# SCUT-BIP-Lab/SplatCo

Measured on AMD Instinct MI355X. Metric: rasterizer fwd+bwd Msplats/s @1080p; PSNR-match vs ref, higher is better.
Workload: dtype f32; 1 GPU; cfg1: 1M synthetic Gaussians (seed 0), 1 view 1920x1080 per GPU, GaussianRasterizer forward+backward, colors_precomp + scale/rotation path; gaussians=1000000, image=1920x1080, visible=1000000, parallelism=1 view per GPU (mv sharding)

## Files before the change

splatco_amd/csrc/binning.hip:

```cpp
#include "common.h"

namespace scr {

template <int THREADS>
__device__ __forceinline__ uint32_t block_exclusive_scan(uint32_t v, uint32_t* lds_waves ,
                                                         uint32_t& block_total) {
    const int lane = threadIdx.x & (WAVE - 1), w = threadIdx.x / WAVE;
    uint32_t inc = v;
#pragma unroll
    for (int d = 1; d < WAVE; d <<= 1) {
        uint32_t n = __shfl_up(inc, d, WAVE);
        if (lane >= d) inc += n;
    }
    if (lane == WAVE - 1) lds_waves[w] = inc;
    __syncthreads();
    uint32_t base = 0, tot = 0;
#pragma unroll
    for (int k = 0; k < THREADS / WAVE; ++k) {
        uint32_t s = lds_waves[k];
        if (k < w) base += s;
        tot += s;
    }
    block_total = tot;
    __syncthreads();
// ... 17 lines not shown
            uint32_t ex = block_exclusive_scan<1024>(v, lds, tot);
            if (i < nblk) block_sums[i] = (uint32_t)carry + ex;
            carry += tot;
            mine += v;
        }
#pragma unroll
        for (int d = WAVE / 2; d > 0; d >>= 1) mine += (unsigned long long)__shfl_down((long long)mine, d, WAVE);
        __syncthreads();
        if ((threadIdx.x & (WAVE - 1)) == 0) wide[threadIdx.x / WAVE] = mine;
        __syncthreads();
        if (threadIdx.x == 0) {
            carry = 0;
            for (int w = 0; w < 1024 / WAVE; ++w) carry += wide[w];
            total[0] = carry;
            if (mailbox) {
                mailbox[0] = carry;
                __threadfence_system();
                mailbox[1] = seq;
            }
        }
    } else {
        uint32_t carry = 0, mx = 0;
        for (uint32_t base = 0; base < tiles; base += 1024) {
            uint32_t i = base + threadIdx.x;
            uint32_t v = i < tiles ? tile_count[i] : 0u, tot;
            uint32_t ex = block_exclusive_scan<1024>(v, lds, tot);
            if (i < tiles) {
                ranges[2 * i] = carry + ex;
                ranges[2 * i + 1] = carry + ex + v;
                cursor[i] = 0;
            }
            carry += tot;
            mx = max(mx, v);
        }
#pragma unroll
        for (int d = 32; d > 0; d >>= 1) mx = max(mx, (uint32_t)__shfl_xor((int)mx, d, WAVE));
        __syncthreads();
        if ((threadIdx.x & 63) == 0) lds[threadIdx.x >> 6] = mx;
        __syncthreads();
        if (threadIdx.x == 0) {
            uint32_t m = 0;
            for (int w = 0; w < 1024 / WAVE; ++w) m = max(m, lds[w]);
            total[1] = m;
            total[2] = 0;
            if (mailbox) {
                mailbox[2] = (unsigned long long)m | (total[3] << 32);
                __threadfence_system();
                mailbox[3] = seq;
            }
        }
    }
}

template <bool LDS_HIST>
__global__ void __launch_bounds__(BIN_THREADS)
scatter_kernel(int64_t P, int gx, int tiles, const float4* __restrict__ rec, uint2* __restrict__ gm_base,
               uint32_t* __restrict__ live_bits, const uint32_t* __restrict__ tiles_touched, const uint32_t* __restrict__ block_prefix,
               uint32_t* __restrict__ point_offsets, const uint32_t* __restrict__ ranges,
               uint32_t* __restrict__ cursor, unsigned long long* __restrict__ keys,
               const unsigned long long* __restrict__ total, unsigned long long cap_instances) {
    extern __shared__ __attribute__((aligned(16))) uint32_t hist[];
    __shared__ uint32_t lds[BIN_THREADS / WAVE + 1];
    if (total[0] > cap_instances) return;
    if (LDS_HIST) {
        for (int t = threadIdx.x; t < tiles; t += BIN_THREADS) hist[t] = 0;
        __syncthreads();
    }
    uint32_t off[BIN_ROUNDS], tts[BIN_ROUNDS], rlo[BIN_ROUNDS], rhi[BIN_ROUNDS], dbits[BIN_ROUNDS];
    uint32_t carry = block_prefix[blockIdx.x];
#pragma unroll
    for (int r = 0; r < BIN_ROUNDS; ++r) {
        const int64_t i = (int64_t)blockIdx.x * BIN_GPW + r * BIN_THREADS + threadIdx.x;
        const uint32_t tt = i < P ? tiles_touched[i] : 0u;
        uint32_t tot;
        off[r] = carry + block_exclusive_scan<BIN_THREADS>(tt, lds, tot);
        carry += tot;
        tts[r] = tt;
        rlo[r] = rhi[r] = dbits[r] = 0;
        if (i < P) point_offsets[i] = off[r] + tt;
        if (tt) {
            const float4 r2 = rec[3 * i + 2];
            dbits[r] = __float_as_uint(r2.y);
            rlo[r] = __float_as_uint(r2.z);
            rhi[r] = __float_as_uint(r2.w);
            const uint32_t x0 = rlo[r] & 0xffff, y0 = rlo[r] >> 16, rw = (rhi[r] & 0xffff) - x0;
            gm_base[i] = make_uint2(off[r] - y0 * rw - x0, rw);
            if (LDS_HIST)
                for (int ty = rlo[r] >> 16; ty < (int)(rhi[r] >> 16); ++ty)
                    for (int tx = rlo[r] & 0xffff; tx < (int)(rhi[r] & 0xffff); ++tx) atomicAdd(&hist[ty * gx + tx], 1u);
        }
    }
    if (LDS_HIST) {
        __syncthreads();
        for (int t = threadIdx.x; t < tiles; t += BIN_THREADS) {
            const uint32_t c = hist[t];
            if (c) hist[t] = ranges[2 * t] + atomicAdd(&cursor[t], c);
        }
        __syncthreads();
    }
#pragma unroll
    for (int r = 0; r < BIN_ROUNDS; ++r) {
        if (!tts[r]) continue;
        const int64_t i = (int64_t)blockIdx.x * BIN_GPW + r * BIN_THREADS + threadIdx.x;
        const uint32_t klo = (uint32_t)i << 4;
        const float4 r0 = rec[3 * i], r1 = rec[3 * i + 1];
        const unsigned long long khi = (unsigned long long)dbits[r] << 32;
        uint32_t live = 0, kbit = 1;
        for (int ty = rlo[r] >> 16; ty < (int)(rhi[r] >> 16); ++ty)
            for (int tx = rlo[r] & 0xffff; tx < (int)(rhi[r] & 0xffff); ++tx) {
                const uint32_t t = (uint32_t)(ty * gx + tx);
                const uint32_t slot = LDS_HIST ? atomicAdd(&hist[t], 1u) : ranges[2 * t] + atomicAdd(&cursor[t], 1u);
                const uint32_t qm = quadrant_mask(r0, r1, tx * TILE, ty * TILE);
                keys[slot] = khi | klo | qm;
                live |= qm ? kbit : 0u;
                kbit <<= 1;
            }
        live_bits[i] = live;
    }
}

template <int D>
__device__ __forceinline__ uint32_t lane_xor(uint32_t v) {
    if constexpr (D == 1) {
        return (uint32_t)__builtin_amdgcn_mov_dpp((int)v, 0xB1, 0xf, 0xf, true);
    } else if constexpr (D == 2) {
        return (uint32_t)__builtin_amdgcn_mov_dpp((int)v, 0x4E, 0xf, 0xf, true);
    } else if constexpr (D == 4) {
        int t = __builtin_amdgcn_update_dpp((int)v, (int)v, 0x104, 0xf, 0x5, false);
        return (uint32_t)__builtin_amdgcn_update_dpp(t, (int)v, 0x114, 0xf, 0xA, false);
    } else if constexpr (D == 8) {
        int t = __builtin_amdgcn_update_dpp((int)v, (int)v, 0x108, 0xf, 0x3, false);
        return (uint32_t)__builtin_amdgcn_update_dpp(t, (int)v, 0x118, 0xf, 0xC, false);
    } else if constexpr (D == 16) {
        auto r = __builtin_amdgcn_permlane16_swap(v, v, false, false);
        return sel(0xFFFF0000FFFF0000ull, r[0], r[1]);
    } else {
        auto r = __builtin_amdgcn_permlane32_swap(v, v, false, false);
        return sel(0xFFFFFFFF00000000ull, r[0], r[1]);
    }
}

constexpr unsigned long long lanes_with_bit_clear(int bit) {
    unsigned long long m = 0;
    for (int l = 0; l < 64; ++l)
        if ((l & bit) == 0) m |= 1ull << l;
// ... 357 lines not shown
    {
        auto keyA = [&](uint32_t i) { return buf[wg_slot((int)i)]; };
        auto keyB = [&](uint32_t j) { return buf[wg_slot((int)(na + j))]; };
        uint32_t a = d0 > nb ? d0 - nb : 0u, b = min(d0, na);
        while (a < b) {
            const uint32_t mid = (a + b) >> 1;
            if (keyA(mid) < keyB(d0 - mid - 1)) a = mid + 1;
            else b = mid;
        }
        uint32_t ia = a, ib = d0 - a;
        unsigned long long x = ia < na ? keyA(ia) : ~0ull, y = ib < nb ? keyB(ib) : ~0ull;
#pragma unroll
        for (int k = 0; k < PER; ++k) {
            const bool takeA = x < y;
            outk[k] = takeA ? x : y;
            if (takeA) {
                ++ia;
                x = ia < na ? keyA(ia) : ~0ull;
            } else {
                ++ib;
                y = ib < nb ? keyB(ib) : ~0ull;
            }
        }
    }
    __syncthreads();
#pragma unroll
    for (int k = 0; k < PER; ++k)
        if (d0 + k < tot) buf[wg_slot((int)(d0 + k))] = outk[k];
    __syncthreads();
    if (pass + 1 == merge_passes_needed(n)) {
        const FinalLists fl{gm_base, point_list, gm_index, qmask, t % gx, t / gx};
        for (uint32_t e = threadIdx.x; e < tot; e += 4 * 256)
            fl.template write_batch<4>(lo + pairbase + s0, e, 256u, tot, [&](uint32_t i, int) { return (uint32_t)buf[wg_slot((int)i)]; });
    } else {
        unsigned long long* out = dst + lo + pairbase + s0;
        for (uint32_t e = threadIdx.x; e < tot; e += 256) out[e] = buf[wg_slot((int)e)];
    }
}

void launch_plan_scans(int64_t P, const KSettings& ks, const GeomView& gv, unsigned long long* mailbox,
                       unsigned long long seq, hipStream_t st) {
    Grid g(ks.H, ks.W);
    uint32_t nb = (uint32_t)((P + BIN_GPW - 1) / BIN_GPW);
    plan_scan_kernel<<<2, 1024, 0, st>>>(nb, gv.block_sums, gv.total, (uint32_t)g.tiles, gv.tile_count,
                                         gv.ranges, gv.cursor, mailbox, seq);
}

void launch_scatter(int64_t P, const KSettings& ks, const GeomView& gv, const BinView& bv, unsigned long long cap_instances,
                    hipStream_t st) {
    if (P <= 0) return;
    Grid g(ks.H, ks.W);
    const unsigned nb = (unsigned)((P + BIN_GPW - 1) / BIN_GPW);
    allow_dynamic_lds((const void*)scatter_kernel<true>, LDS_HIST_MAX_TILES * 4);
    if (g.tiles <= LDS_HIST_MAX_TILES)
        scatter_kernel<true><<<nb, BIN_THREADS, (size_t)g.tiles * 4, st>>>(
            P, g.gx, g.tiles, gv.rec, gv.gm_base, gv.live_bits, gv.tiles_touched, gv.block_sums, gv.point_offsets, gv.ranges,
            gv.cursor, bv.keys, gv.total, cap_instances);
    else
        scatter_kernel<false><<<nb, BIN_THREADS, 0, st>>>(
            P, g.gx, g.tiles, gv.rec, gv.gm_base, gv.live_bits, gv.tiles_touched, gv.block_sums, gv.point_offsets, gv.ranges,
            gv.cursor, bv.keys, gv.total, cap_instances);
}

void launch_tile_sort(const KSettings& ks, const GeomView& gv, const BinView& bv, int64_t max_tile_instances,
                      bool with_gm_index, hipStream_t st) {
    uint32_t* const gm_index = with_gm_index ? bv.gm_index : nullptr;
    Grid g(ks.H, ks.W);
    const unsigned gt = (unsigned)xcd_grid(g.tiles);
    if (max_tile_instances <= 0) return;
    tile_sort_wave_kernel<<<gt, 64, 0, st>>>(g.tiles, g.gx, gv.ranges, bv.keys, gv.gm_base, bv.point_list, gm_index,
                                             bv.qmask);
    if (max_tile_instances <= WAVE_SORT_MAX) return;
    const unsigned chunks = (unsigned)((max_tile_instances + WG_SORT_MAX - 1) / WG_SORT_MAX);
    const size_t lds = (size_t)(WG_SORT_MAX + WG_SORT_MAX / 16) * 8;
    allow_dynamic_lds((const void*)tile_sort_wg_kernel, lds);
    tile_sort_wg_kernel<<<dim3(gt, chunks), WG_SORT_THREADS, lds, st>>>(g.tiles, g.gx, gv.ranges, bv.keys, gv.gm_base, bv.point_list,
                                                                        gm_index, bv.qmask);
    if (chunks <= 1) return;
    unsigned passes = 0;
    while ((1u << passes) < chunks) ++passes;
    const unsigned segs = (unsigned)((max_tile_instances + MP_SEG - 1) / MP_SEG);
    for (unsigned p = 0; p < passes; ++p) {
        const unsigned long long* src = (p & 1u) ? bv.keys2 : bv.keys;
        unsigned long long* dst = (p & 1u) ? bv.keys : bv.keys2;
        tile_merge_path_kernel<<<dim3(gt, segs), 256, 0, st>>>(g.tiles, g.gx, p, gv.ranges, src, dst, gv.gm_base,
                                                               bv.point_list, gm_index, bv.qmask);
    }
}

}
```

splatco_amd/csrc/capi.hip:

```cpp
#include <stdarg.h>
#include <stdio.h>
#include <string.h>

#include "common.h"
#include "adam.h"
#include "tv.h"
#include <chrono>
#include <map>
#include <mutex>
#include <utility>
#include <cstring>

using namespace scr;

static thread_local char g_err[512] = "";
namespace scr {
int g_force_deep_lists = -1;

void allow_dynamic_lds(const void* kernel, size_t bytes) {
    if (bytes <= 65536) return;
    static std::mutex mu;
    static std::map<std::pair<int, const void*>, size_t> granted;
    int dev = 0;
    (void)hipGetDevice(&dev);
    std::lock_guard<std::mutex> lk(mu);
    size_t& have = granted[{dev, kernel}];
    if (bytes <= have) return;
    if (hipFuncSetAttribute(kernel, hipFuncAttributeMaxDynamicSharedMemorySize, (int)bytes) == hipSuccess) have = bytes;
    (void)hipGetLastError();
}
}

static int fail(const char* fmt, ...) {
    va_list ap;
    va_start(ap, fmt);
    vsnprintf(g_err, sizeof(g_err), fmt, ap);
    va_end(ap);
    return 1;
}

#define HIP_TRY(expr)                                                                      \
    do {                                                                                   \
        hipError_t e_ = (expr);                                                            \
        if (e_ != hipSuccess) return fail("%s failed: %s", #expr, hipGetErrorString(e_)); \
    } while (0)

#define CHECK_LAUNCH(name, debug, st)                                                      \
    do {                                                                                   \
        hipError_t e_ = hipGetLastError();                                                 \
        if (e_ != hipSuccess) return fail("launch of %s failed: %s", name, hipGetErrorString(e_)); \
        if (debug) {                                                                       \
            e_ = hipStreamSynchronize(st);                                                 \
            if (e_ != hipSuccess) return fail("%s faulted: %s", name, hipGetErrorString(e_)); \
        }                                                                                  \
    } while (0)

#include <dlfcn.h>
#include <atomic>
#include <vector>
namespace {
struct ProfRec { int idx; hipEvent_t a, b; };
unsigned g_prof_mask = 0;
unsigned g_prof_stride = 1;
unsigned g_prof_seen[32] = {};
std::vector<ProfRec> g_prof_recs;
std::vector<hipEvent_t> g_prof_pool;
hipEvent_t prof_event() {
    hipEvent_t e;
    if (!g_prof_pool.empty()) { e = g_prof_pool.back(); g_prof_pool.pop_back(); return e; }
    (void)hipEventCreate(&e);
// ... 372 lines not shown
    if (check_settings(settings)) return 1;
    if (P < 0) return fail("P < 0");
    const bool camera = dL_dviewmatrix || dL_dprojmatrix || dL_dcampos;
    if (P == 0) {
        if (dL_dviewmatrix) HIP_TRY(hipMemsetAsync(dL_dviewmatrix, 0, 16 * sizeof(float), (hipStream_t)stream));
        if (dL_dprojmatrix) HIP_TRY(hipMemsetAsync(dL_dprojmatrix, 0, 16 * sizeof(float), (hipStream_t)stream));
        if (dL_dcampos) HIP_TRY(hipMemsetAsync(dL_dcampos, 0, 3 * sizeof(float), (hipStream_t)stream));
        return 0;
    }
    if (plan_flags & ~(int64_t)(SCR_PLAN_NONFINITE_COLOUR | SCR_PLAN_LARGE_RECTS)) return fail("plan_flags %lld: not a value scr_forward_plan returned", (long long)plan_flags);
    if (!geom_buf || !binning_buf || !image_buf || !dL_dcolor || !scratch) return fail("NULL buffer");
    if (!means3D || !radii || !dL_dmeans3D || !dL_dmeans2D || !dL_dopacity) return fail("NULL argument");
    if (shs ? !dL_dsh : !dL_dcolors) return fail("colour gradient output missing");
    if (cov3D_precomp ? !dL_dcov3D : !(dL_dscales && dL_drotations && scales && rotations))
        return fail("covariance gradient output missing");
    hipStream_t st = (hipStream_t)stream;
    KSettings ks = ksettings(settings);
    GeomView gv = geom_view(geom_buf, P, ks.H, ks.W);
    BinView bv = bin_view((void*)binning_buf, I, 0);
    ImgView iv = img_view(image_buf, ks.H, ks.W);
    static std::atomic<unsigned long long> stamp_counter{0x5ca1ab1e00000000ull};
    const unsigned long long stamp = ++stamp_counter;
    float* const grad_z = (I > 0 && (dL_ddepth || dL_dalpha)) ? (float*)((char*)scratch + grad_rec_bytes(I)) : nullptr;
    float* const cam_partials = camera ? (float*)((char*)scratch + grad_rec_bytes(I) + grad_z_bytes(I)) : nullptr;
    if (settings->debug) {
        unsigned long long dev_flags = 0;
        HIP_TRY(hipMemcpyAsync(&dev_flags, gv.total + 3, 8, hipMemcpyDeviceToHost, st));
        HIP_TRY(hipStreamSynchronize(st));
        if ((long long)dev_flags != (long long)plan_flags)
            return fail("plan_flags %lld passed to scr_backward, but the forward pass of this geom_buf raised %llu", (long long)plan_flags, dev_flags);
    }
    if (I > 0) {
        launch_zero_far_records(P, gv, (GradRec*)scratch, grad_z, st);
        CHECK_LAUNCH("zero_far_records_kernel", settings->debug, st);
        { ProfScope ps_(SCR_PROF_BLEND_BACKWARD, st);
          launch_blend_backward(ks, gv, bv, iv, dL_dcolor, dL_ddepth, dL_dalpha, (GradRec*)scratch, grad_z, stamp, deep_lists(I, Grid(ks.H, ks.W).tiles),
                                record_flags(I, Grid(ks.H, ks.W).tiles), (plan_flags & SCR_PLAN_NONFINITE_COLOUR) != 0, st); }
        CHECK_LAUNCH("blend_backward_kernel", settings->debug, st);
    }
    { ProfScope ps_(SCR_PROF_PREPROCESS_BACKWARD, st);
      launch_preprocess_backward(P, M, means3D, scales, rotations, cov3D_precomp, shs, ks, radii, gv, bv,
                                 (const GradRec*)scratch, grad_z, iv.cut_key, stamp, record_flags(I, Grid(ks.H, ks.W).tiles), dL_dmeans3D, dL_dmeans2D, shs ? nullptr : dL_dcolors,
                                 shs ? dL_dsh : nullptr, dL_dopacity, cov3D_precomp ? nullptr : dL_dscales,
                                 cov3D_precomp ? nullptr : dL_drotations, cov3D_precomp ? dL_dcov3D : nullptr, cam_partials, st); }
    CHECK_LAUNCH("preprocess_backward_kernel", settings->debug, st);
    if (camera) {
        launch_camera_grad_finish(P, cam_partials, dL_dviewmatrix, dL_dprojmatrix, dL_dcampos, st);
        CHECK_LAUNCH("camera_grad_finish_kernel", settings->debug, st);
    }
    return 0;
}

int scr_debug_force_deep_lists(int mode) {
    if (mode < -1 || mode > 1) return fail("scr_debug_force_deep_lists: -1 (automatic), 0 or 1");
    scr::g_force_deep_lists = mode;
    return 0;
}

int scr_debug_get(int which, int64_t P, int64_t I, int32_t H, int32_t W, const void* geom_buf,
                  const void* binning_buf, const void* image_buf, void* out, void* stream) {
    SCR_MARK_FN;
    hipStream_t st = (hipStream_t)stream;
    Grid g(H, W);
    const void* src = nullptr;
    size_t bytes = 0;
    if (which <= SCR_DBG_RANGES || which == SCR_DBG_SPLAT_RECORDS) {
        if (!geom_buf) return fail("geom_buf is NULL");
        GeomView gv = geom_view((void*)geom_buf, P, H, W);
        if (which == SCR_DBG_TILES_TOUCHED) { src = gv.tiles_touched; bytes = (size_t)P * 4; }
        else if (which == SCR_DBG_POINT_OFFSETS) { src = gv.point_offsets; bytes = (size_t)P * 4; }
        else if (which == SCR_DBG_RANGES) { src = gv.ranges; bytes = (size_t)g.tiles * 8; }
        else { src = gv.rec; bytes = (size_t)P * REC_F * 4; }
    } else if (which == SCR_DBG_POINT_LIST) {
        if (!binning_buf) return fail("binning_buf is NULL");
        src = bin_view((void*)binning_buf, I, 0).point_list;
        bytes = (size_t)I * 4;
    } else if (which == SCR_DBG_QMASK || which == SCR_DBG_GM_INDEX) {
        if (!binning_buf) return fail("binning_buf is NULL");
        BinView bv = bin_view((void*)binning_buf, I, 0);
        if (which == SCR_DBG_GM_INDEX && deep_lists(I, g.tiles))
            return fail("gm_index is not materialised for deep tile lists (I > 8192 per tile on average)");
        src = which == SCR_DBG_QMASK ? (const void*)bv.qmask : (const void*)bv.gm_index;
        bytes = which == SCR_DBG_QMASK ? (size_t)I : (size_t)I * 4;
    } else if (which == SCR_DBG_N_CONTRIB || which == SCR_DBG_FINAL_T) {
        if (!image_buf) return fail("image_buf is NULL");
        ImgView iv = img_view((void*)image_buf, H, W);
        src = which == SCR_DBG_N_CONTRIB ? (const void*)iv.n_contrib : (const void*)iv.final_T;
        bytes = (size_t)H * W * 4;
    } else {
        return fail("unknown debug selector %d", which);
    }
    if (bytes) HIP_TRY(hipMemcpyAsync(out, src, bytes, hipMemcpyDeviceToDevice, st));
    return 0;
}

static inline size_t expand_nwg(int64_t n) { return (size_t)((n + 1023) / 1024); }

size_t scr_expand_scratch_bytes(int64_t n) { return align_up((expand_nwg(n) + 1) * 4) + 256; }

int scr_expand_plan(int64_t n, const float* neural_opacity, void* scratch, int64_t* num_selected_host,
                    void* stream) {
    SCR_MARK_FN;
    if (!num_selected_host) return fail("num_selected_host is NULL");
    *num_selected_host = 0;
    if (n < 0) return fail("n < 0");
    if (n == 0) return 0;
    if (!neural_opacity || !scratch) return fail("NULL argument");
    if (n >= (1ll << 31)) return fail("more than 2^31 candidates");
// ... 793 lines not shown
```

splatco_amd/csrc/common.h:

```cpp
#pragma once
#include <hip/hip_runtime.h>
#include <stdint.h>

#include "../../include/splatco_raster.h"

namespace scr {

__host__ __device__ __forceinline__ uint32_t sat_add_u32(uint32_t a, uint32_t b) {
    const uint32_t s = a + b;
    return s < a ? 0xFFFFFFFFu : s;
}


constexpr int TILE = SCR_TILE;
constexpr int TILE_PIX = TILE * TILE;
constexpr int WAVE = 64;
constexpr int NUM_XCD = 8;
constexpr int PRE_BLOCK = 256;
constexpr int BIN_THREADS = 1024;
constexpr int BIN_ROUNDS = 4;
constexpr int BIN_GPW = BIN_THREADS * BIN_ROUNDS;
constexpr int LDS_HIST_MAX_TILES = 40000;
constexpr int ID_BITS = 28;
constexpr int WG_SORT_MAX = 8192;
constexpr int REC_F = 12;
constexpr int GRAD_F = 9;

inline __host__ __device__ size_t align_up(size_t x, size_t a = 256) { return (x + a - 1) / a * a; }

struct Grid {
    int W, H, gx, gy, tiles;
    __host__ __device__ Grid(int H_, int W_)
        : W(W_), H(H_), gx((W_ + TILE - 1) / TILE), gy((H_ + TILE - 1) / TILE), tiles(gx * gy) {}
};

struct GeomView {
    float4* rec;
    uint32_t* tiles_touched;
    uint32_t* point_offsets;
    uint8_t* clamped;
    uint2* gm_base;
    uint32_t* live_bits;
    uint8_t* has_rec;
    uint32_t* block_sums;
    uint32_t* tile_count;
    uint32_t* ranges;
    uint32_t* cursor;
    int64_t P;
    unsigned long long* total;
    size_t bytes;
};

inline __host__ GeomView geom_view(void* base, int64_t P, int H, int W) {
    Grid g(H, W);
    char* p = (char*)base;
    size_t off = 0;
    GeomView v;
    auto take = [&](size_t n) { char* q = p ? p + off : nullptr; off += align_up(n); return q; };
    size_t nblk = (size_t)((P + BIN_GPW - 1) / BIN_GPW);
    v.rec = (float4*)take((size_t)P * REC_F * 4);
    v.tiles_touched = (uint32_t*)take((size_t)P * 4);
    v.point_offsets = (uint32_t*)take((size_t)P * 4);
    v.clamped = (uint8_t*)take((size_t)P);
    v.gm_base = (uint2*)take((size_t)P * 8);
    v.live_bits = (uint32_t*)take((size_t)P * 4);
    v.has_rec = (uint8_t*)take((size_t)P);
    v.block_sums = (uint32_t*)take((nblk + 1) * 4);
    v.tile_count = (uint32_t*)take((size_t)g.tiles * 4);
    v.ranges = (uint32_t*)take((size_t)g.tiles * 8);
    v.cursor = (uint32_t*)take((size_t)g.tiles * 4);
    v.total = (unsigned long long*)take(128);
    v.bytes = off;
    v.P = P;
    return v;
}

extern int g_force_deep_lists;
inline __host__ bool deep_lists(int64_t I, int tiles) {
    return g_force_deep_lists >= 0 ? g_force_deep_lists != 0 : I > (int64_t)8192 * tiles;
}

constexpr int FLAGS_MIN_MEAN = 2048;
inline __host__ bool record_flags(int64_t I, int tiles) {
    return g_force_deep_lists >= 0 ? g_force_deep_lists != 0 : I > (int64_t)FLAGS_MIN_MEAN * tiles;
}

struct BinView {
    unsigned long long* keys;
    uint32_t* point_list;
    uint32_t* gm_index;
    uint8_t* qmask;
    unsigned long long* keys2;
    size_t bytes;
};

inline __host__ BinView bin_view(void* base, int64_t I, int64_t max_tile_instances) {
    char* p = (char*)base;
    size_t off = 0;
    BinView v;
    auto take = [&](size_t n) { char* q = p ? p + off : nullptr; off += align_up(n); return q; };
    size_t n = (size_t)(I > 0 ? I : 1);
    v.keys = (unsigned long long*)take(n * 8);
    v.point_list = (uint32_t*)take(n * 4);
    v.gm_index = (uint32_t*)take(n * 4);
    v.qmask = (uint8_t*)take(n);
    const bool merge = max_tile_instances > WG_SORT_MAX;
    v.keys2 = merge ? (unsigned long long*)take(n * 8) : nullptr;
    v.bytes = off;
    return v;
}

struct __attribute__((packed, aligned(4))) GradQuad { float x, y, z, w; };
struct __attribute__((packed, aligned(4))) GradRec { GradQuad a, b; float c; };
static_assert(sizeof(GradRec) == 36, "36-byte gradient records");
inline __host__ size_t grad_rec_bytes(int64_t I) { return align_up((size_t)(I > 0 ? I : 1) * sizeof(GradRec)); }
inline __host__ size_t grad_z_bytes(int64_t I) { return align_up((size_t)(I > 0 ? I : 1) * sizeof(float)); }

struct ImgView {
    float* final_T;
    uint32_t* n_contrib;
    unsigned long long* cut_key;
    size_t bytes;
};

// ... 311 lines not shown
```

splatco_amd/csrc/preprocess.hip:

```cpp
#include "common.h"

namespace scr {

struct Proj {
    float t[3];
    float hx, hy, hw;
    float cov[6];
    float txc, tyc;
    bool clx, cly;
    float T[2][3];
    float a, b, c;
};

__device__ __forceinline__ void xform3(const float* __restrict__ M, float x, float y, float z, int i,
                                       float& out) {
    out = ((M[i] * x + M[4 + i] * y) + M[8 + i] * z) + M[12 + i];
}

__device__ __forceinline__ void rotmat(const float q[4], float R[3][3]) {
    float r = q[0], x = q[1], y = q[2], z = q[3];
    R[0][0] = 1.0f - 2.0f * (y * y + z * z);
    R[0][1] = 2.0f * (x * y - r * z);
    R[0][2] = 2.0f * (x * z + r * y);
    R[1][0] = 2.0f * (x * y + r * z);
// ... 122 lines not shown
}

__global__ void __launch_bounds__(256) mark_visible_kernel(int64_t P, const float* __restrict__ means3D,
                                                           const float* __restrict__ V,
                                                           uint8_t* __restrict__ out) {
    int64_t i = (int64_t)blockIdx.x * 256 + threadIdx.x;
    if (i >= P) return;
    float tz;
    xform3(V, means3D[3 * i], means3D[3 * i + 1], means3D[3 * i + 2], 2, tz);
    out[i] = tz > 0.2f;
}

__device__ static const float SH_C0 = 0.28209479177387814f;
__device__ static const float SH_C1 = 0.4886025119029199f;
__device__ static const float SH_C2[5] = {1.0925484305920792f, -1.0925484305920792f, 0.31539156525252005f,
                                          -1.0925484305920792f, 0.5462742152960396f};
__device__ static const float SH_C3[7] = {-0.5900435899266435f, 2.890611442640554f, -0.4570457994644658f,
                                          0.3731763325901154f,  -0.4570457994644658f, 1.445305721320277f,
                                          -0.5900435899266435f};

__device__ __forceinline__ void sh_to_rgb(int deg, const float* __restrict__ sh, float x, float y,
                                          float z, float rgb[3], uint8_t& clampbits) {
    clampbits = 0;
#pragma unroll
    for (int c = 0; c < 3; ++c) {
#define SHV(k) sh[(k)*3 + c]
        float res = SH_C0 * SHV(0);
        if (deg > 0) {
            res = res - SH_C1 * y * SHV(1) + SH_C1 * z * SHV(2) - SH_C1 * x * SHV(3);
            if (deg > 1) {
                float xx = x * x, yy = y * y, zz = z * z, xy = x * y, yz = y * z, xz = x * z;
                res = res + SH_C2[0] * xy * SHV(4) + SH_C2[1] * yz * SHV(5) +
                      SH_C2[2] * (2.0f * zz - xx - yy) * SHV(6) + SH_C2[3] * xz * SHV(7) +
                      SH_C2[4] * (xx - yy) * SHV(8);
                if (deg > 2) {
                    res = res + SH_C3[0] * y * (3.0f * xx - yy) * SHV(9) + SH_C3[1] * xy * z * SHV(10) +
                          SH_C3[2] * y * (4.0f * zz - xx - yy) * SHV(11) +
                          SH_C3[3] * z * (2.0f * zz - 3.0f * xx - 3.0f * yy) * SHV(12) +
                          SH_C3[4] * x * (4.0f * zz - xx - yy) * SHV(13) + SH_C3[5] * z * (xx - yy) * SHV(14) +
                          SH_C3[6] * x * (xx - 3.0f * yy) * SHV(15);
                }
            }
        }
#undef SHV
        res += 0.5f;
        if (res < 0.0f) {
            clampbits |= (uint8_t)(1u << c);
            res = 0.0f;
        }
        rgb[c] = res;
    }
}

template <bool LDS_HIST>
__global__ void __launch_bounds__(BIN_THREADS)
preprocess_kernel(int64_t P, int M, const float* __restrict__ means3D, const float* __restrict__ scales,
                  const float* __restrict__ rotations, const float* __restrict__ cov3D,
                  const float* __restrict__ opacities, const float* __restrict__ shs,
                  const float* __restrict__ colors, KSettings ks, int tiles, float4* __restrict__ rec,
                  uint32_t* __restrict__ tiles_touched, uint8_t* __restrict__ clamped,
                  uint32_t* __restrict__ block_sums, uint32_t* __restrict__ tile_count,
                  int32_t* __restrict__ radii, unsigned long long* __restrict__ plan_flags) {
    extern __shared__ __attribute__((aligned(16))) uint32_t hist[];
    __shared__ uint32_t wave_sum[BIN_THREADS / WAVE];
    if (LDS_HIST) {
        for (int t = threadIdx.x; t < tiles; t += BIN_THREADS) hist[t] = 0;
        __syncthreads();
    }
    const int gx = (ks.W + TILE - 1) / TILE;
    uint32_t tsum = 0;
    for (int r = 0; r < BIN_ROUNDS; ++r) {
        const int64_t i = (int64_t)blockIdx.x * BIN_GPW + r * BIN_THREADS + threadIdx.x;
        if (i >= P) break;
        uint32_t tt = 0;
        Proj ps;
        Foot ft;
        bool vis = project(i, means3D, scales, rotations, cov3D, ks, ps, ft);
        if (vis) {
            float a = ps.a, b = ps.b, c = ps.c;
            float Qxx = c * ft.det_inv, Qxy = -b * ft.det_inv, Qyy = a * ft.det_inv;
            float rgb[3];
            uint8_t cb = 0;
            if (colors) {
                rgb[0] = colors[3 * i];
                rgb[1] = colors[3 * i + 1];
                rgb[2] = colors[3 * i + 2];
            } else {
                float dx = means3D[3 * i] - ks.campos[0], dy = means3D[3 * i + 1] - ks.campos[1],
                      dz = means3D[3 * i + 2] - ks.campos[2];
                float n = sqrtf((dx * dx + dy * dy) + dz * dz);
                sh_to_rgb(ks.sh_degree, shs + (size_t)i * M * 3, dx / n, dy / n, dz / n, rgb, cb);
            }
            if (clamped) clamped[i] = cb;
            tt = (uint32_t)((ft.rmaxx - ft.rminx) * (ft.rmaxy - ft.rminy));
            const unsigned long long w_nf = lanes(nonfinite3(rgb[0], rgb[1], rgb[2])), w_big = lanes(tt > 32u);
            if ((w_nf | w_big) != 0ull) {
                const unsigned long long active = lanes(true);
                if ((int)__builtin_amdgcn_mbcnt_hi(~0u, __builtin_amdgcn_mbcnt_lo(~0u, 0u)) == __builtin_ctzll(active))
                    atomicOr(plan_flags, (unsigned long long)((w_nf ? SCR_PLAN_NONFINITE_COLOUR : 0) | (w_big ? SCR_PLAN_LARGE_RECTS : 0)));
            }
            uint32_t rlo = (uint32_t)ft.rminx | ((uint32_t)ft.rminy << 16);
            uint32_t rhi = (uint32_t)ft.rmaxx | ((uint32_t)ft.rmaxy << 16);
            rec[3 * i + 0] = make_float4(ft.mx, ft.my, -0.5f * Qxx, -Qxy);
            rec[3 * i + 1] = make_float4(-0.5f * Qyy, opacities[i], rgb[0], rgb[1]);
            rec[3 * i + 2] = make_float4(rgb[2], ps.t[2], __uint_as_float(rlo), __uint_as_float(rhi));
            radii[i] = ft.radius;
            for (int ty = ft.rminy; ty < ft.rmaxy; ++ty)
                for (int tx = ft.rminx; tx < ft.rmaxx; ++tx) {
                    if (LDS_HIST) atomicAdd(&hist[ty * gx + tx], 1u);
                    else atomicAdd(&tile_count[ty * gx + tx], 1u);
                }
        } else {
            radii[i] = 0;
            if (clamped) clamped[i] = 0;
        }
        tiles_touched[i] = tt;
        tsum = sat_add_u32(tsum, tt);
    }
    uint32_t s = tsum;
#pragma unroll
    for (int d = WAVE / 2; d > 0; d >>= 1) s = sat_add_u32(s, (uint32_t)__shfl_down(s, d, WAVE));
    if ((threadIdx.x & (WAVE - 1)) == 0) wave_sum[threadIdx.x / WAVE] = s;
    __syncthreads();
    if (threadIdx.x == 0) {
        uint32_t tot = 0;
#pragma unroll
        for (int w = 0; w < BIN_THREADS / WAVE; ++w) tot = sat_add_u32(tot, wave_sum[w]);
        block_sums[blockIdx.x] = tot;
    }
    if (LDS_HIST)
        for (int t = threadIdx.x; t < tiles; t += BIN_THREADS) {
            const uint32_t c = hist[t];
            if (c) atomicAdd(&tile_count[t], c);
        }
}

constexpr int CAM_VALUES = 27, CAM_ROW = 32;
__device__ __forceinline__ void cam_workgroup_sum(const float* v, float* __restrict__ row) {
    __shared__ float wave_part[PRE_BLOCK / WAVE][CAM_ROW];
#pragma unroll
    for (int k = 0; k < CAM_VALUES; ++k) {
        float s = v[k];
#pragma unroll
        for (int d = WAVE / 2; d > 0; d >>= 1) s += __shfl_down(s, d, WAVE);
        if ((threadIdx.x & (WAVE - 1)) == 0) wave_part[threadIdx.x / WAVE][k] = s;
    }
    __syncthreads();
    if (threadIdx.x < CAM_ROW) {
        float tot = 0.0f;
        if (threadIdx.x < CAM_VALUES) {
#pragma unroll
            for (int w = 0; w < PRE_BLOCK / WAVE; ++w) tot += wave_part[w][threadIdx.x];
        }
        row[threadIdx.x] = tot;
    }
}

template <bool AUX, bool POSE>
__global__ void __launch_bounds__(PRE_BLOCK, 1)
preprocess_backward_kernel(int64_t P, int M, const float* __restrict__ means3D,
                           const float* __restrict__ scales, const float* __restrict__ rotations,
                           const float* __restrict__ cov3D, const float* __restrict__ shs, KSettings ks,
                           const int32_t* __restrict__ radii, const uint32_t* __restrict__ tiles_touched,
                           const uint32_t* __restrict__ point_offsets, const uint32_t* __restrict__ live_bits,
                           const uint8_t* __restrict__ has_rec, const uint8_t* __restrict__ clamped,
                           const float4* __restrict__ rec, const GradRec* __restrict__ grad_rec,
                           const unsigned long long* __restrict__ cut_key, unsigned long long stamp, int tiles,
                           float* __restrict__ dL_dmeans3D, float* __restrict__ dL_dmeans2D,
                           float* __restrict__ dL_dcolors, float* __restrict__ dL_dsh,
                           float* __restrict__ dL_dopacity, float* __restrict__ dL_dscales,
                           float* __restrict__ dL_drotations, float* __restrict__ dL_dcov3D,
                           const float* __restrict__ grad_z, float* __restrict__ cam_partials) {
    int64_t i = (int64_t)blockIdx.x * PRE_BLOCK + threadIdx.x;
    bool inb = true;
    if (POSE) {
        inb = i < P;
        if (!inb) i = P - 1;
    } else if (i >= P) return;
    float cg[POSE ? CAM_VALUES : 1] = {};
    float gm[3] = {0, 0, 0}, gm2[3] = {0, 0, 0}, gcol[3] = {0, 0, 0}, gop = 0, gs[3] = {0, 0, 0},
          gq[4] = {0, 0, 0, 0}, g6[6] = {0, 0, 0, 0, 0, 0};
    bool vis = radii[i] > 0;
    if (POSE && !inb) vis = false;
    if (has_rec && !has_rec[i]) vis = false;
    const float4 r2 = rec[3 * i + 2];
    Proj ps;
    Foot ft;
// ... 299 lines not shown
                          float* __restrict__ dL_dproj, float* __restrict__ dL_dcampos) {
    constexpr int SLICES = CAM_FINISH_THREADS / CAM_ROW;
    __shared__ double part[SLICES][CAM_ROW];
    const int col = threadIdx.x % CAM_ROW, slice = threadIdx.x / CAM_ROW;
    double acc = 0.0;
    int64_t r = slice;
    for (; r + 7 * SLICES < rows; r += 8 * SLICES) {
        float x[8];
#pragma unroll
        for (int j = 0; j < 8; ++j) x[j] = partials[(r + j * SLICES) * CAM_ROW + col];
#pragma unroll
        for (int j = 0; j < 8; ++j) acc += (double)x[j];
    }
    for (; r < rows; r += SLICES) acc += (double)partials[r * CAM_ROW + col];
    part[slice][col] = acc;
    __syncthreads();
    const int t = threadIdx.x;
    if (t >= 35) return;
    auto total = [&](int k) {
        double s = 0.0;
        for (int w = 0; w < SLICES; ++w) s += part[w][k];
        return (float)s;
    };
    if (t < 16) {
        const int c = t >> 2, j = t & 3;
        if (dL_dview) dL_dview[t] = j < 3 ? total(3 * c + j) : 0.0f;
    } else if (t < 32) {
        const int c = (t - 16) >> 2, j = t & 3;
        if (dL_dproj) dL_dproj[t - 16] = j != 2 ? total(12 + 3 * c + (j == 3 ? 2 : j)) : 0.0f;
    } else if (dL_dcampos) {
        dL_dcampos[t - 32] = total(24 + (t - 32));
    }
}

static inline unsigned nblk(int64_t P, int per) { return (unsigned)((P + per - 1) / per); }

void launch_filter(int64_t P, const float* means3D, const float* scales, const float* rotations,
                   const float* cov3D, const KSettings& ks, int32_t* radii, hipStream_t st) {
    if (P <= 0) return;
    filter_kernel<<<nblk(P, 256), 256, 0, st>>>(P, means3D, scales, rotations, cov3D, ks, radii);
}

void launch_mark_visible(int64_t P, const float* means3D, const float* view, uint8_t* out, hipStream_t st) {
    if (P <= 0) return;
    mark_visible_kernel<<<nblk(P, 256), 256, 0, st>>>(P, means3D, view, out);
}

void launch_preprocess(int64_t P, int M, const float* means3D, const float* scales, const float* rotations,
                       const float* cov3D, const float* opacities, const float* shs, const float* colors,
                       const KSettings& ks, const GeomView& gv, int32_t* radii, hipStream_t st) {
    if (P <= 0) return;
    Grid g(ks.H, ks.W);
    allow_dynamic_lds((const void*)preprocess_kernel<true>, LDS_HIST_MAX_TILES * 4);
    if (g.tiles <= LDS_HIST_MAX_TILES)
        preprocess_kernel<true><<<nblk(P, BIN_GPW), BIN_THREADS, (size_t)g.tiles * 4, st>>>(
            P, M, means3D, scales, rotations, cov3D, opacities, shs, colors, ks, g.tiles, gv.rec, gv.tiles_touched,
            shs ? gv.clamped : nullptr, gv.block_sums, gv.tile_count, radii, gv.total + 3);
    else
        preprocess_kernel<false><<<nblk(P, BIN_GPW), BIN_THREADS, 0, st>>>(
            P, M, means3D, scales, rotations, cov3D, opacities, shs, colors, ks, g.tiles, gv.rec, gv.tiles_touched,
            shs ? gv.clamped : nullptr, gv.block_sums, gv.tile_count, radii, gv.total + 3);
}

void launch_preprocess_backward(int64_t P, int M, const float* means3D, const float* scales,
                                const float* rotations, const float* cov3D, const float* shs,
                                const KSettings& ks, const int32_t* radii, const GeomView& gv,
                                const BinView& bv, const GradRec* grad_rec, const float* grad_z,
                                const unsigned long long* cut_key, unsigned long long stamp, bool deep, float* dL_dmeans3D,
                                float* dL_dmeans2D, float* dL_dcolors, float* dL_dsh, float* dL_dopacity,
                                float* dL_dscales, float* dL_drotations, float* dL_dcov3D, float* cam_partials,
                                hipStream_t st) {
    if (P <= 0) return;
    auto kernel = cam_partials ? (grad_z ? preprocess_backward_kernel<true, true> : preprocess_backward_kernel<false, true>)
                               : (grad_z ? preprocess_backward_kernel<true, false> : preprocess_backward_kernel<false, false>);
    kernel<<<nblk(P, PRE_BLOCK), PRE_BLOCK, 0, st>>>(
        P, M, means3D, scales, rotations, cov3D, shs, ks, radii, gv.tiles_touched, gv.point_offsets, gv.live_bits,
        deep ? gv.has_rec : nullptr, gv.clamped, gv.rec, grad_rec, cut_key, stamp, Grid(ks.H, ks.W).tiles, dL_dmeans3D, dL_dmeans2D, dL_dcolors, dL_dsh, dL_dopacity,
        dL_dscales, dL_drotations, dL_dcov3D, grad_z, cam_partials);
}

size_t camera_partials_bytes(int64_t P) { return align_up((size_t)(P > 0 ? nblk(P, PRE_BLOCK) : 1) * CAM_ROW * sizeof(float)); }

void launch_camera_grad_finish(int64_t P, const float* cam_partials, float* dL_dview, float* dL_dproj, float* dL_dcampos,
                               hipStream_t st) {
    camera_grad_finish_kernel<<<1, CAM_FINISH_THREADS, 0, st>>>(P > 0 ? (int64_t)nblk(P, PRE_BLOCK) : 0, cam_partials, dL_dview,
                                                                 dL_dproj, dL_dcampos);
}

__global__ void __launch_bounds__(256) zero_far_records_kernel(int64_t P, const unsigned long long* __restrict__ total,
                                                               const uint32_t* __restrict__ tiles_touched,
                                                               const uint32_t* __restrict__ point_offsets, uint32_t* __restrict__ rec_words,
                                                               float* __restrict__ grad_z) {
    if ((total[3] & (unsigned long long)SCR_PLAN_LARGE_RECTS) == 0ull) return;
    const int lane = threadIdx.x & 63;
    for (int64_t base = (int64_t)blockIdx.x * 256 + (threadIdx.x & ~63); base < P; base += (int64_t)gridDim.x * 256) {
        const int64_t i = base + lane;
        const uint32_t n = i < P ? tiles_touched[i] : 0u;
        const uint32_t end = (i < P && n > 32u) ? point_offsets[i] : 0u;
        unsigned long long big = lanes(n > 32u);
        while (big) {
            const int src = __builtin_ctzll(big);
            big &= big - 1;
            const uint32_t n_s = (uint32_t)__shfl((int)n, src, WAVE), end_s = (uint32_t)__shfl((int)end, src, WAVE);
            const size_t w0 = (size_t)(end_s - n_s + 32u) * GRAD_F, w1 = (size_t)end_s * GRAD_F;
            for (size_t w = w0 + lane; w < w1; w += WAVE) rec_words[w] = 0u;
            if (grad_z)
                for (size_t w = (size_t)(end_s - n_s + 32u) + lane; w < (size_t)end_s; w += WAVE) grad_z[w] = 0.0f;
        }
    }
}
void launch_zero_far_records(int64_t P, const GeomView& gv, GradRec* grad_rec, float* grad_z, hipStream_t st) {
    if (P <= 0) return;
    const int64_t want = (P + 255) / 256;
    zero_far_records_kernel<<<(unsigned)(want < 2048 ? want : 2048), 256, 0, st>>>(P, gv.total, gv.tiles_touched, gv.point_offsets, (uint32_t*)grad_rec, grad_z);
// ... 24 lines not shown
```

Measured before the change: 1084 Msplats/s.

## Record per-block tile run starts in preprocess to skip scatter histogram pass

Preprocess now saves, per block and tile, the offset returned by its atomicAdd into the global tile counts as a run-start table. Scatter seeds its LDS slot table from ranges plus this run start instead of rebuilding the per-tile histogram with LDS atomics and claiming slots with global cursor atomics. The trade is a table of blocks×tiles words (capped at 32MB) written and read through global memory, plus writing zero rows for every tile. A debug mode forces the old count pass.

New measurement: 1089 Msplats/s, median of 6. Within noise of the previous version (+0.4%).

```diff
diff --git a/splatco_amd/csrc/binning.hip b/splatco_amd/csrc/binning.hip
--- a/splatco_amd/csrc/binning.hip
+++ b/splatco_amd/csrc/binning.hip
@@ -93,17 +93,23 @@
     }
 }
 
-template <bool LDS_HIST>
+template <bool LDS_HIST, bool RUNS = false>
 __global__ void __launch_bounds__(BIN_THREADS)
 scatter_kernel(int64_t P, int gx, int tiles, const float4* __restrict__ rec, uint2* __restrict__ gm_base,
                uint32_t* __restrict__ live_bits, const uint32_t* __restrict__ tiles_touched, const uint32_t* __restrict__ block_prefix,
                uint32_t* __restrict__ point_offsets, const uint32_t* __restrict__ ranges,
                uint32_t* __restrict__ cursor, unsigned long long* __restrict__ keys,
-               const unsigned long long* __restrict__ total, unsigned long long cap_instances) {
+               const unsigned long long* __restrict__ total, unsigned long long cap_instances,
+               const uint32_t* __restrict__ run_start) {
+    static_assert(LDS_HIST || !RUNS, "the run starts become the LDS slot table");
     extern __shared__ __attribute__((aligned(16))) uint32_t hist[];
     __shared__ uint32_t lds[BIN_THREADS / WAVE + 1];
     if (total[0] > cap_instances) return;
-    if (LDS_HIST) {
+    if (RUNS) {
+        const uint32_t* __restrict__ row = run_start + (size_t)blockIdx.x * (size_t)tiles;
+        const uint2* __restrict__ seg = (const uint2*)ranges;
+        for (int t = threadIdx.x; t < tiles; t += BIN_THREADS) hist[t] = seg[t].x + row[t];
+    } else if (LDS_HIST) {
         for (int t = threadIdx.x; t < tiles; t += BIN_THREADS) hist[t] = 0;
         __syncthreads();
     }
@@ -126,12 +132,14 @@
             rhi[r] = __float_as_uint(r2.w);
             const uint32_t x0 = rlo[r] & 0xffff, y0 = rlo[r] >> 16, rw = (rhi[r] & 0xffff) - x0;
             gm_base[i] = make_uint2(off[r] - y0 * rw - x0, rw);
-            if (LDS_HIST)
+            if (LDS_HIST && !RUNS)
                 for (int ty = rlo[r] >> 16; ty < (int)(rhi[r] >> 16); ++ty)
                     for (int tx = rlo[r] & 0xffff; tx < (int)(rhi[r] & 0xffff); ++tx) atomicAdd(&hist[ty * gx + tx], 1u);
         }
     }
-    if (LDS_HIST) {
+    if (RUNS) {
+        __syncthreads();
+    } else if (LDS_HIST) {
         __syncthreads();
         for (int t = threadIdx.x; t < tiles; t += BIN_THREADS) {
             const uint32_t c = hist[t];
@@ -595,14 +603,19 @@
     Grid g(ks.H, ks.W);
     const unsigned nb = (unsigned)((P + BIN_GPW - 1) / BIN_GPW);
     allow_dynamic_lds((const void*)scatter_kernel<true>, LDS_HIST_MAX_TILES * 4);
-    if (g.tiles <= LDS_HIST_MAX_TILES)
+    allow_dynamic_lds((const void*)scatter_kernel<true, true>, LDS_HIST_MAX_TILES * 4);
+    if (gv.run_start)
+        scatter_kernel<true, true><<<nb, BIN_THREADS, (size_t)g.tiles * 4, st>>>(
+            P, g.gx, g.tiles, gv.rec, gv.gm_base, gv.live_bits, gv.tiles_touched, gv.block_sums, gv.point_offsets, gv.ranges,
+            gv.cursor, bv.keys, gv.total, cap_instances, gv.run_start);
+    else if (g.tiles <= LDS_HIST_MAX_TILES)
         scatter_kernel<true><<<nb, BIN_THREADS, (size_t)g.tiles * 4, st>>>(
             P, g.gx, g.tiles, gv.rec, gv.gm_base, gv.live_bits, gv.tiles_touched, gv.block_sums, gv.point_offsets, gv.ranges,
-            gv.cursor, bv.keys, gv.total, cap_instances);
+            gv.cursor, bv.keys, gv.total, cap_instances, nullptr);
     else
         scatter_kernel<false><<<nb, BIN_THREADS, 0, st>>>(
             P, g.gx, g.tiles, gv.rec, gv.gm_base, gv.live_bits, gv.tiles_touched, gv.block_sums, gv.point_offsets, gv.ranges,
-            gv.cursor, bv.keys, gv.total, cap_instances);
+            gv.cursor, bv.keys, gv.total, cap_instances, nullptr);
 }
 
 void launch_tile_sort(const KSettings& ks, const GeomView& gv, const BinView& bv, int64_t max_tile_instances,
diff --git a/splatco_amd/csrc/capi.hip b/splatco_amd/csrc/capi.hip
--- a/splatco_amd/csrc/capi.hip
+++ b/splatco_amd/csrc/capi.hip
@@ -16,6 +16,7 @@
 static thread_local char g_err[512] = "";
 namespace scr {
 int g_force_deep_lists = -1;
+int g_force_count_pass = 0;
 
 void allow_dynamic_lds(const void* kernel, size_t bytes) {
     if (bytes <= 65536) return;
@@ -494,8 +495,9 @@
 }
 
 int scr_debug_force_deep_lists(int mode) {
-    if (mode < -1 || mode > 1) return fail("scr_debug_force_deep_lists: -1 (automatic), 0 or 1");
-    scr::g_force_deep_lists = mode;
+    if (mode < -1 || mode > 2) return fail("scr_debug_force_deep_lists: -1 (automatic), 0, 1 or 2 (no run table)");
+    scr::g_force_deep_lists = mode == 2 ? -1 : mode;
+    scr::g_force_count_pass = mode == 2;
     return 0;
 }
 
diff --git a/splatco_amd/csrc/common.h b/splatco_amd/csrc/common.h
--- a/splatco_amd/csrc/common.h
+++ b/splatco_amd/csrc/common.h
@@ -21,6 +21,7 @@
 constexpr int BIN_ROUNDS = 4;
 constexpr int BIN_GPW = BIN_THREADS * BIN_ROUNDS;
 constexpr int LDS_HIST_MAX_TILES = 40000;
+constexpr size_t RUN_TABLE_MAX_BYTES = (size_t)32 << 20;
 constexpr int ID_BITS = 28;
 constexpr int WG_SORT_MAX = 8192;
 constexpr int REC_F = 12;
@@ -46,10 +47,18 @@
     uint32_t* tile_count;
     uint32_t* ranges;
     uint32_t* cursor;
+    uint32_t* run_start;
     int64_t P;
     unsigned long long* total;
     size_t bytes;
 };
+
+extern int g_force_count_pass;
+inline __host__ size_t run_table_bytes(int64_t P, int tiles) {
+    if (g_force_count_pass || P <= 0 || tiles > LDS_HIST_MAX_TILES) return 0;
+    const size_t bytes = (size_t)((P + BIN_GPW - 1) / BIN_GPW) * (size_t)tiles * 4;
+    return bytes <= RUN_TABLE_MAX_BYTES ? bytes : 0;
+}
 
 inline __host__ GeomView geom_view(void* base, int64_t P, int H, int W) {
     Grid g(H, W);
@@ -70,6 +79,8 @@
     v.ranges = (uint32_t*)take((size_t)g.tiles * 8);
     v.cursor = (uint32_t*)take((size_t)g.tiles * 4);
     v.total = (unsigned long long*)take(128);
+    const size_t table = run_table_bytes(P, g.tiles);
+    v.run_start = table ? (uint32_t*)take(table) : nullptr;
     v.bytes = off;
     v.P = P;
     return v;
diff --git a/splatco_amd/csrc/preprocess.hip b/splatco_amd/csrc/preprocess.hip
--- a/splatco_amd/csrc/preprocess.hip
+++ b/splatco_amd/csrc/preprocess.hip
@@ -198,7 +198,7 @@
     }
 }
 
-template <bool LDS_HIST>
+template <bool LDS_HIST, bool RUNS = false>
 __global__ void __launch_bounds__(BIN_THREADS)
 preprocess_kernel(int64_t P, int M, const float* __restrict__ means3D, const float* __restrict__ scales,
                   const float* __restrict__ rotations, const float* __restrict__ cov3D,
@@ -206,7 +206,9 @@
                   const float* __restrict__ colors, KSettings ks, int tiles, float4* __restrict__ rec,
                   uint32_t* __restrict__ tiles_touched, uint8_t* __restrict__ clamped,
                   uint32_t* __restrict__ block_sums, uint32_t* __restrict__ tile_count,
-                  int32_t* __restrict__ radii, unsigned long long* __restrict__ plan_flags) {
+                  int32_t* __restrict__ radii, unsigned long long* __restrict__ plan_flags,
+                  uint32_t* __restrict__ run_start) {
+    static_assert(LDS_HIST || !RUNS, "the run table is written from the LDS histogram");
     extern __shared__ __attribute__((aligned(16))) uint32_t hist[];
     __shared__ uint32_t wave_sum[BIN_THREADS / WAVE];
     if (LDS_HIST) {
@@ -274,11 +276,28 @@
         for (int w = 0; w < BIN_THREADS / WAVE; ++w) tot = sat_add_u32(tot, wave_sum[w]);
         block_sums[blockIdx.x] = tot;
     }
-    if (LDS_HIST)
+    if (RUNS) {
+        uint32_t* __restrict__ row = run_start + (size_t)blockIdx.x * (size_t)tiles;
+        for (int t0 = threadIdx.x; t0 < tiles; t0 += 4 * BIN_THREADS) {
+            uint32_t old[4];
+#pragma unroll
+            for (int u = 0; u < 4; ++u) {
+                const int t = t0 + u * BIN_THREADS;
+                const uint32_t c = t < tiles ? hist[t] : 0u;
+                old[u] = c ? atomicAdd(&tile_count[t], c) : 0u;
+            }
+#pragma unroll
+            for (int u = 0; u < 4; ++u) {
+                const int t = t0 + u * BIN_THREADS;
+                if (t < tiles) row[t] = old[u];
+            }
+        }
+    } else if (LDS_HIST) {
         for (int t = threadIdx.x; t < tiles; t += BIN_THREADS) {
             const uint32_t c = hist[t];
             if (c) atomicAdd(&tile_count[t], c);
         }
+    }
 }
 
 constexpr int CAM_VALUES = 27, CAM_ROW = 32;
@@ -684,14 +703,19 @@
     if (P <= 0) return;
     Grid g(ks.H, ks.W);
     allow_dynamic_lds((const void*)preprocess_kernel<true>, LDS_HIST_MAX_TILES * 4);
-    if (g.tiles <= LDS_HIST_MAX_TILES)
+    allow_dynamic_lds((const void*)preprocess_kernel<true, true>, LDS_HIST_MAX_TILES * 4);
+    if (gv.run_start)
+        preprocess_kernel<true, true><<<nblk(P, BIN_GPW), BIN_THREADS, (size_t)g.tiles * 4, st>>>(
+            P, M, means3D, scales, rotations, cov3D, opacities, shs, colors, ks, g.tiles, gv.rec, gv.tiles_touched,
+            shs ? gv.clamped : nullptr, gv.block_sums, gv.tile_count, radii, gv.total + 3, gv.run_start);
+    else if (g.tiles <= LDS_HIST_MAX_TILES)
         preprocess_kernel<true><<<nblk(P, BIN_GPW), BIN_THREADS, (size_t)g.tiles * 4, st>>>(
             P, M, means3D, scales, rotations, cov3D, opacities, shs, colors, ks, g.tiles, gv.rec, gv.tiles_touched,
-            shs ? gv.clamped : nullptr, gv.block_sums, gv.tile_count, radii, gv.total + 3);
+            shs ? gv.clamped : nullptr, gv.block_sums, gv.tile_count, radii, gv.total + 3, nullptr);
     else
         preprocess_kernel<false><<<nblk(P, BIN_GPW), BIN_THREADS, 0, st>>>(
             P, M, means3D, scales, rotations, cov3D, opacities, shs, colors, ks, g.tiles, gv.rec, gv.tiles_touched,
-            shs ? gv.clamped : nullptr, gv.block_sums, gv.tile_count, radii, gv.total + 3);
+            shs ? gv.clamped : nullptr, gv.block_sums, gv.tile_count, radii, gv.total + 3, nullptr);
 }
 
 void launch_preprocess_backward(int64_t P, int M, const float* means3D, const float* scales,
```
